# Fagear/SDVPCMdecoder

Measured on AMD Instinct MI355X. Metric: decoded video frames/sec (720x486 STC-007), binarize+bit-extract+CRC, bit-exact vs CPU, higher is better.
Workload: dtype u8; 1 GPU; configs[1]: 10000-frame synthetic STC-007 NTSC 720x486 batch per GPU resident in HBM, Binarizer mode 2, noise sigma 4.0, binarize+bit-extract+CRC only; decoded_words_match_generator=True

## Files before the change

### sdvpcmdecoder_amd/csrc/stc007_device.h

```cpp
#ifndef SDV_STC007_DEVICE_H
#define SDV_STC007_DEVICE_H

#include "../../include/sdvpcm.h"

#ifndef SDV_EMU
#include <hip/hip_runtime.h>
#endif

#define SDV_MAX_WIDTH 1536
#ifndef SDV_BATCH_LINES
#define SDV_BATCH_LINES 2
#endif
#ifndef SDV_NT_RECORDS
#define SDV_NT_RECORDS 1
#endif
#ifndef SDV_CAPTURE_D
#define SDV_CAPTURE_D 4
#endif
#ifndef SDV_RB_GENERAL
#define SDV_RB_GENERAL 1
#endif
#ifndef SDV_PREFETCH_ITERS
#define SDV_PREFETCH_ITERS 1
#endif
// ... 2015 lines not shown
    const int lane = lane_id();
    uint16_t w[9];
    bits_to_words(fb.s_lo, fb.s_hi, w);
    w[8] = fb.calc_crc;

    K1_T(t_bk0);
    const bool even_line = (line_num % 2) == 0;
    const bool doubled = a.doubled != 0;
    bool forced_bad = false;
    if (v.field_state == FIELD_NEW) v.field_state = FIELD_UNSAFE;
    v.good_coords_in_field++;
    v.q_line_length = (uint16_t)a.width;
    if (a.check_line_copy) {
        if (v.field_state == FIELD_UNSAFE) {
            b.in_coord.doubled = doubled;
            if (kMeasure) bin_set_bw_levels(b, ps, black, white);
            if (ps.en_first_line_dup) forced_bad = true;
        } else {
            uint8_t diff = words_diff_bit_count(w, v.last_words);
            Line t; t.m2 = a.m2_format != 0; for (int i = 0; i < 6; i++) t.words[i] = w[i];
            if (!stc_is_almost_silent(t) && diff <= (BITS_DATA / BIT_DIFF_THRES_DIV)) { forced_bad = true; if (!even_line) v.q_dup_odd++; else v.q_dup_even++; }
        }
    }
    K1_T(t_bk1);
    {
        uint32_t key = coords_key(b.in_coord.start, b.in_coord.stop);
        SDV_WAVE_SYNC();
        if (lane == 0) {
            if (v.n_last == COORD_HISTORY_DEPTH) for (int i = 0; i < COORD_HISTORY_DEPTH - 1; i++) lds.lv_keys[i] = lds.lv_keys[i + 1];
            lds.lv_keys[v.n_last == COORD_HISTORY_DEPTH ? COORD_HISTORY_DEPTH - 1 : v.n_last] = key;
        }
        if (v.n_last < COORD_HISTORY_DEPTH) v.n_last++;
        SDV_WAVE_SYNC();
        fv_keys[v.nfv++] = key;
        K1_T(t_bk2);
        K1_ADD(16, t_bk0, t_bk1); K1_ADD(17, t_bk1, t_bk2);
        if (a.coordinate_damper && (v.n_last > (COORD_HISTORY_DEPTH / 2))) {
            Coords target; coords_clear(target);
            uint32_t k;
            if (median_keys(lds.lv_keys, v.n_last, &k)) target = key_to_coords(k, false);
            if (!coords_valid(target)) target = v.frame_avg;
            if (coords_valid(target)) {
                int16_t ds = (int16_t)(b.in_coord.start - target.start), de = (int16_t)(b.in_coord.stop - target.stop);
                uint8_t in_delta = (uint8_t)(((uint8_t)(g.psm / 128u)) * 3);
                if (((int)ds <= -(int)in_delta) || ((int)ds >= (int)in_delta) || ((int)de <= -(int)in_delta) || ((int)de >= (int)in_delta)) forced_bad = true;
            }
        }
        K1_T(t_bk2b);
        K1_ADD(18, t_bk2, t_bk2b);
    }
    K1_T(t_bk3);
    if (!forced_bad) { b.in_coord.doubled = doubled; if (kMeasure) bin_set_bw_levels(b, ps, black, white); }
    else { if (!even_line) v.q_bad_odd++; else v.q_bad_even++; }
    v.field_state = FIELD_INIT;
    if (!even_line) { v.q_odd++; v.q_pcm_odd++; } else { v.q_even++; v.q_pcm_even++; }
    v.pcm_lines_in_field++;
    for (int i = 0; i < 8; i++) v.last_words[i] = w[i];
    v.line_in_field_cnt++;
    b.line_length = (uint16_t)a.width;

    if (lane == 0) {
        sdv_line_rec r;
        r.frame_number = frame_no; r.line_number = line_num;
        for (int i = 0; i < 9; i++) r.words[i] = w[i];
        r.calc_crc = fb.calc_crc;
        r.data_start = b.in_coord.start; r.data_stop = b.in_coord.stop;
        r.marker_start_bg_coord = 0; r.marker_start_ed_coord = 0; r.marker_stop_ed_coord = found_sp_ed;
        r.black_level = black; r.white_level = white; r.ref_low = fb.ref_low; r.ref_level = b.in_ref; r.ref_high = fb.ref_high;
        r.hysteresis_depth = fb.h; r.shift_stage = fb.s; r.service_type = SDV_SRV_NO;
        r.mark_st_stage = MARK_ST_START; r.mark_ed_stage = found_mark_ed;
        r.flags = (uint8_t)(SDV_LF_BY_EXT_TUNE | SDV_LF_BW_SET | (forced_bad ? SDV_LF_FORCED_BAD : SDV_LF_CRC_VALID) | (doubled ? SDV_LF_FROM_DOUBLED : 0));
        r.word_state = forced_bad ? 0 : (uint8_t)(SDV_WS_WORD_CRC | SDV_WS_WORD_VALID);
        *rec = r;
    }
    K1_T(t_bk4);
    K1_ADD(19, t_bk3, t_bk4);
    return true;
}

struct BatchLaneOut { uint64_t s_lo, s_hi; uint16_t crc; };
#ifdef SDV_EMU
__device__ __forceinline__ uint32_t write_lane(uint32_t old, uint32_t val, int lane) { return lane_id() == lane ? val : old; }
__device__ __forceinline__ uint8_t stream_load_u8(const uint8_t *p) { return *p; }
#define SDV_ISSUE_AFTER8(oa, ob, m0, m1, m2, m3, m4, m5, m6, m7) ((void)0)
#else
__device__ __forceinline__ uint8_t stream_load_u8(const uint8_t *p) { return __builtin_nontemporal_load(p); }
#define SDV_ISSUE_AFTER8(oa, ob, m0, m1, m2, m3, m4, m5, m6, m7) \
    asm volatile("" : "+s"(oa), "+s"(ob) : "s"(m0), "s"(m1), "s"(m2), "s"(m3), "s"(m4), "s"(m5), "s"(m6), "s"(m7))
extern "C" __device__ uint32_t sdv_llvm_writelane(uint32_t val, uint32_t lane, uint32_t old) __asm("llvm.amdgcn.writelane.i32");
__device__ __forceinline__ uint32_t write_lane(uint32_t old, uint32_t val, int lane) { return sdv_llvm_writelane(val, (uint32_t)lane, old); }
#endif
struct CaptureRaw { uint32_t a0, a1, a2, a3, b0, b1, b2, b3; };
__device__ __forceinline__ void capture_park(CaptureRaw &r, uint64_t a_lo, uint64_t a_hi, uint64_t b_lo, uint64_t b_hi, int j)
{
    r.a0 = write_lane(r.a0, (uint32_t)a_lo, j); r.a1 = write_lane(r.a1, (uint32_t)(a_lo >> 32), j);
    r.a2 = write_lane(r.a2, (uint32_t)a_hi, j); r.a3 = write_lane(r.a3, (uint32_t)(a_hi >> 32), j);
    r.b0 = write_lane(r.b0, (uint32_t)b_lo, j); r.b1 = write_lane(r.b1, (uint32_t)(b_lo >> 32), j);
    r.b2 = write_lane(r.b2, (uint32_t)b_hi, j); r.b3 = write_lane(r.b3, (uint32_t)(b_hi >> 32), j);
}
template <bool kAnyPattern = false>
__device__ inline bool capture_solve(const CaptureRaw &r, BatchLaneOut &o)
{
    const uint64_t a_lo = (uint64_t)r.a0 | ((uint64_t)r.a1 << 32), a_hi = (uint64_t)r.a2 | ((uint64_t)r.a3 << 32);
    const uint64_t b_lo = (uint64_t)r.b0 | ((uint64_t)r.b1 << 32), b_hi = (uint64_t)r.b2 | ((uint64_t)r.b3 << 32);
    const uint64_t e_lo = ~(a_lo ^ b_lo), e_hi = ~(a_hi ^ b_hi), t_lo = a_lo & ~b_lo, t_hi = a_hi & ~b_hi;
    const uint64_t pt_lo = prefix_xor64(t_lo), pt_hi = prefix_xor64(t_hi) ^ ((__popcll(t_lo) & 1) ? ~0ull : 0ull);
    const uint64_t u_lo = ((a_lo & b_lo) ^ pt_lo) & e_lo, u_hi = ((a_hi & b_hi) ^ pt_hi) & e_hi;
    const uint64_t x_lo = u_lo | ~e_lo, x_hi = u_hi | ~e_hi;
    const uint64_t y_lo = x_lo + u_lo, y_hi = x_hi + u_hi + ((y_lo < x_lo) ? 1ull : 0ull);
    const uint64_t s_lo = ((((y_lo ^ x_lo) & ~e_lo) | u_lo) ^ pt_lo), s_hi = ((((y_hi ^ x_hi) & ~e_hi) | u_hi) ^ pt_hi);
    uint32_t crc = 0;
#pragma unroll
    for (int j = 0; j < 16; j++) crc |= (uint32_t)((__popcll(s_lo & c_crc.klo[j]) + __popcll(s_hi & c_crc.khi[j])) & 1) << j;
    crc ^= c_crc.init;
    o.s_lo = s_lo; o.s_hi = s_hi; o.crc = (uint16_t)crc;
    return (uint16_t)crc == rev16((uint32_t)((s_hi >> 48) & 0xFFFF)) && (kAnyPattern || !ctrl_block_maybe(s_lo));
}

struct SolveOut { uint32_t d0, d1, d2, d3, crc_reads; };
#ifndef SDV_EMU
__device__ __attribute__((noinline)) SolveOut capture_solve_call(uint32_t a0, uint32_t a1, uint32_t a2, uint32_t a3, uint32_t b0, uint32_t b1, uint32_t b2, uint32_t b3)
#else
__device__ inline SolveOut capture_solve_call(uint32_t a0, uint32_t a1, uint32_t a2, uint32_t a3, uint32_t b0, uint32_t b1, uint32_t b2, uint32_t b3)
#endif
{
    CaptureRaw c; c.a0 = a0; c.a1 = a1; c.a2 = a2; c.a3 = a3; c.b0 = b0; c.b1 = b1; c.b2 = b2; c.b3 = b3;
    BatchLaneOut o;
    const bool reads = capture_solve<true>(c, o);
    SolveOut r; r.d0 = (uint32_t)o.s_lo; r.d1 = (uint32_t)(o.s_lo >> 32); r.d2 = (uint32_t)o.s_hi; r.d3 = (uint32_t)(o.s_hi >> 32);
    r.crc_reads = (uint32_t)o.crc | (reads ? 0x10000u : 0u);
    return r;
}

struct BatchLane { uint32_t d0, d1, d2, d3, meta; };

__device__ inline bool batch_eligible(const FrameArgs &a, const WaveLds &lds, const V2D &v, const Geo &g)
{
    if (!fast_eligible(a, v.bin)) return false;
    if (v.n_last != COORD_HISTORY_DEPTH) return false;
    uint32_t key = coords_key(v.bin.in_coord.start, v.bin.in_coord.stop);
    bool differs = (lane_id() < COORD_HISTORY_DEPTH) && (lds.lv_keys[lane_id() < COORD_HISTORY_DEPTH ? lane_id() : 0] != key);
    if (__ballot(differs) != 0ull) return false;
    if (a.coordinate_damper) {
        uint32_t psm = (uint32_t)((int)v.bin.in_coord.stop - (int)v.bin.in_coord.start);
        psm = (psm * 128u + BITS_BETWEEN / 2) / BITS_BETWEEN;
        if ((uint8_t)(((uint8_t)(psm / 128u)) * 3) == 0) return false;
    }
    return true;
}

enum { REC_STAGE_OFS = 5120, REC_STAGE_BYTES = 1024 };
static_assert(REC_STAGE_OFS >= ((SDV_MAX_HEIGHT / 2 + 63) / 64) * 4 * 64 * sizeof(uint32_t), "the parked lines of a field of SDV_MAX_HEIGHT / 2 lines end in front of the record stage");
static_assert(REC_STAGE_OFS >= SDV_PX_BYTES && REC_STAGE_OFS + REC_STAGE_BYTES <= offsetof(WaveLds, crc_stats), "the record stage lies behind the staged scanlines and in front of the histories");
#ifndef SDV_COALESCED_RECORDS
#define SDV_COALESCED_RECORDS 1
#endif

__device__ inline void batch_finish(const FrameArgs &a, WaveLds &lds, V2D &v, const BatchLane &bl, int n, uint32_t frame_no, uint16_t first_line_num,
                                    uint32_t *fv_keys, sdv_line_rec *rec, bool write_keys = true, uint4 *direct_dst = nullptr, int *n_forced = nullptr)
{
    const sdv_bin_preset &ps = a.preset;
    Bin &b = v.bin;
    const int lane = lane_id();
    const bool active = lane < n;
    const bool doubled = a.doubled != 0;
    const bool even_line = (first_line_num % 2) == 0;
    uint64_t s_lo = (uint64_t)bl.d0 | ((uint64_t)bl.d1 << 32), s_hi = (uint64_t)bl.d2 | ((uint64_t)bl.d3 << 32);
    uint16_t w[8];
    bits_to_words(s_lo, s_hi, w);
// ... 170 lines not shown
            v2d_give_up(a, lds, f);
            return;
        } else {
            uint16_t ln = 0;
            if (f == a.new_file_frame) { v2d_service_line(v, a, lds, wl, frame_no, 0, SDV_SRV_NEW_FILE); emit_record(wl, rec++); }
            for (int field = 0; field < 2; field++) {
                const int nl = field == 0 ? (a.height + 1) / 2 : a.height / 2;
                for (int i = 0; i < nl; i++) {
                    ln = (uint16_t)(field + 1 + 2 * i);
                    SDV_SLOW_CTX(c);
                    SDV_WAVE_SYNC();
                    if (!sc_args_set) { c.a = a; sc_args_set = true; }
                    c.v = v;
                    SDV_WAVE_SYNC();
                    empty_line(&c, &lds, frame_no, ln, fv_keys, fi_keys, rec++);
                    SDV_WAVE_SYNC();
                    v = c.v;
                    v2d_make_uniform(v);
                }
                ln = (uint16_t)(ln + 2);
                v2d_service_line(v, a, lds, wl, frame_no, ln, SDV_SRV_END_FIELD);
                emit_record(wl, rec++);
            }
            ln = (uint16_t)(ln + 2);
            v2d_service_line(v, a, lds, wl, frame_no, ln, SDV_SRV_END_FRAME);
            v2d_end_frame(v, a, lds, frame_no, fv_keys, fi_keys, &a.stats[f]);
            emit_record(wl, rec++);
            v2d_store_state(v, lds, &a.states_out[f], a);
            return;
        }
    }
    if (f == a.end_file_frame) {
        uint16_t ln = 0;
        for (int field = 0; field < 2; field++) {
            const int nl = field == 0 ? (a.height + 1) / 2 : a.height / 2;
            for (int i = 0; i < nl; i++) {
                ln = (uint16_t)(field + 1 + 2 * i);
                v2d_service_line(v, a, lds, wl, frame_no, ln, SDV_SRV_FILLER);
                emit_record(wl, rec++);
            }
            ln = (uint16_t)(ln + 2);
            v2d_service_line(v, a, lds, wl, frame_no, ln, SDV_SRV_END_FIELD);
            emit_record(wl, rec++);
        }
        ln = (uint16_t)(ln + 2);
        v2d_service_line(v, a, lds, wl, frame_no, ln, SDV_SRV_END_FILE);
        emit_record(wl, rec++);
        ln = (uint16_t)(ln + 2);
        v2d_service_line(v, a, lds, wl, frame_no, ln, SDV_SRV_END_FRAME);
        v2d_end_frame(v, a, lds, frame_no, fv_keys, fi_keys, &a.stats[f]);
        emit_record(wl, rec++);
        v2d_store_state(v, lds, &a.states_out[f], a);
        return;
    }
    if (f == a.new_file_frame) { v2d_service_line(v, a, lds, wl, frame_no, 0, SDV_SRV_NEW_FILE); emit_record(wl, rec++); }
    if (kFat && a.tc_hdr && lane == 0) a.tc_hdr[2 * f] = 0;
    if (!kLean && kMeet && a.tc_hdr) {
        tc_on = true;
        tc_prev = uniu(a.tc_hdr[2 * f]); tc_prev_n = uniu(a.tc_hdr[2 * f + 1]);
        if (tc_prev > 2u || tc_prev_n > (uint32_t)TC_FINAL) tc_prev = 0;
        tc_wbuf = tc_prev == 1u ? 1 : 0;
        tc_wr = a.tc_snaps + ((size_t)f * 2u + (size_t)tc_wbuf) * TC_ENTRIES;
        if (tc_prev) {
            tc_rd = a.tc_snaps + ((size_t)f * 2u + (size_t)(tc_prev - 1u)) * TC_ENTRIES;
            tc_my_pos = lane < (int)tc_prev_n ? (tc_rd[lane].d[18] & 0xFFFFu) : (uint32_t)TC_POS_NONE;
            tc_rd_keys = (tc_prev == 2u ? a.tc_keys : a.scratch) + (size_t)f * 2u * (size_t)a.height;
        }
        if (tc_wbuf) { fv_keys = a.tc_keys + (size_t)f * 2u * (size_t)a.height; fi_keys = fv_keys + a.height; }
        SDV_WAVE_SYNC();
        if (lane == 0) a.tc_hdr[2 * f] = 0;
    }
    const int n_field[2] = { (a.height + 1) / 2, a.height / 2 };
    RowPrefetch pf;
    pf.v0 = uint4{0, 0, 0, 0}; pf.v1 = uint4{0, 0, 0, 0};
    for (int u = 0; u < SDV_ROWQ; u++) { pf.vq[u] = uint4{0, 0, 0, 0}; pf.rowq[u] = frame; }
    pf.nq = 0;
    pf.vec = ((((uintptr_t)frame) | (uintptr_t)a.row_stride) & 15) == 0 && a.width >= 16;
    { int nvec = a.width >> 4; pf.i0 = lane < nvec ? lane : (nvec > 0 ? nvec - 1 : 0); }
    row_prefetch(pf, frame, a.width);
    const size_t row_step = 2 * a.row_stride;
    uint16_t line_num = 0;
    int start_field = 0, start_idx = 0;
    bool all_captured = false; uint32_t captured_key = 0;
    bool frame_direct = false;
    bool sweep_pending = false;
    bool used_general = false;
#ifdef SDV_K1_STAMPS
    int n_slow_lines = 0;
#endif
    if (kLean && pf.vec && a.width <= 1024 && (a.width & 15) == 0 && n_field[1] > 0 && (uint64_t)a.row_stride * (uint64_t)a.height < (1ull << 31) &&
        batch_eligible(a, lds, v, geo)) {
        const FastPre pre = fast_pre(a, v.bin, geo);
        if (pre.ok) {
            K1_T(t_cap);
            const int n0 = n_field[0], n1 = n_field[1];
            const int n_chunks = (n0 + 63) / 64;
            uint32_t *park = (uint32_t *)lds.px;
            uint64_t ok0_packed = 0, ok1_packed = 0;
            enum { HOLD_CHUNKS = (SDV_MAX_HEIGHT / 2 + 63) / 64 };
            uint32_t hold[HOLD_CHUNKS][4];
#pragma unroll
            for (int u = 0; u < HOLD_CHUNKS; u++) hold[u][0] = hold[u][1] = hold[u][2] = hold[u][3] = 0;
            int n_done = 0;
            const uint32_t rs = (uint32_t)a.row_stride;
            const uint32_t lo = pre.ref_low, hi = pre.ref_high;
            const uint32_t x0 = (uint32_t)pre.x0, x1 = (uint32_t)pre.x1;
            constexpr int D = SDV_CAPTURE_D;
            static_assert(64 % D == 0, "the prefetch queue must stay aligned with the 64-line chunks");
            auto pair_offsets = [&](int kn, uint32_t &oa, uint32_t &ob) {
                const uint32_t k = (uint32_t)(kn < n0 ? kn : n0 - 1);
                oa = 2u * k * rs; ob = (int)k < n1 ? oa + rs : oa; };
            uint8_t q[D][4];
#pragma unroll
            for (int d = 0; d < D; d++) {
                uint32_t oa, ob; pair_offsets(d, oa, ob);
                q[d][0] = stream_load_u8(frame + (oa + x0)); q[d][1] = stream_load_u8(frame + (oa + x1));
                q[d][2] = stream_load_u8(frame + (ob + x0)); q[d][3] = stream_load_u8(frame + (ob + x1));
            }
            bool whole = true;
            for (int c = 0; c < n_chunks && whole; c++) {
                const int cn0 = n0 - 64 * c < 64 ? n0 - 64 * c : 64, cn1 = n1 - 64 * c < 64 ? (n1 - 64 * c > 0 ? n1 - 64 * c : 0) : 64;
                CaptureRaw r0, r1;
                r0.a0 = r0.a1 = r0.a2 = r0.a3 = r0.b0 = r0.b1 = r0.b2 = r0.b3 = 0;
                r1 = r0;
                for (int j0 = 0; j0 < cn0; j0 += D) {
#pragma unroll
                    for (int d = 0; d < D; d++) {
                        const int j = j0 + d;
                        const uint8_t p0 = q[d][0], p1 = q[d][1], p2 = q[d][2], p3 = q[d][3];
                        const uint64_t aA_lo = __ballot(p0 > lo), bA_lo = __ballot(p0 >= hi), aA_hi = __ballot(p1 > lo), bA_hi = __ballot(p1 >= hi);
                        const uint64_t aB_lo = __ballot(p2 > lo), bB_lo = __ballot(p2 >= hi), aB_hi = __ballot(p3 > lo), bB_hi = __ballot(p3 >= hi);
                        {
                            uint32_t oa, ob; pair_offsets(64 * c + j + D, oa, ob);
                            SDV_ISSUE_AFTER8(oa, ob, aA_lo, bA_lo, aA_hi, bA_hi, aB_lo, bB_lo, aB_hi, bB_hi);
                            q[d][0] = stream_load_u8(frame + (oa + x0)); q[d][1] = stream_load_u8(frame + (oa + x1));
                            q[d][2] = stream_load_u8(frame + (ob + x0)); q[d][3] = stream_load_u8(frame + (ob + x1));
                        }
                        capture_park(r0, aA_lo, aA_hi, bA_lo, bA_hi, j);
                        capture_park(r1, aB_lo, aB_hi, bB_lo, bB_hi, j);
                    }
                }
                K1_T(t_s0);
                BatchLaneOut o0, o1;
                const bool ok0 = capture_solve(r0, o0), ok1 = capture_solve(r1, o1);
                const uint64_t okm0 = __ballot(ok0 || lane >= cn0), okm1 = __ballot(ok1 || lane >= cn1);
                const int n_ok0 = okm0 == ~0ull ? cn0 : (__ffsll((unsigned long long)~okm0) - 1);
                const int n_ok1 = okm1 == ~0ull ? cn1 : (__ffsll((unsigned long long)~okm1) - 1);
                ok0_packed |= (uint64_t)n_ok0 << (7 * c); ok1_packed |= (uint64_t)n_ok1 << (7 * c);
                K1_T(t_s1);
                K1_ADD(5, t_s0, t_s1);
                park[(c * 4 + 0) * 64 + lane] = (uint32_t)o1.s_lo; park[(c * 4 + 1) * 64 + lane] = (uint32_t)(o1.s_lo >> 32);
                park[(c * 4 + 2) * 64 + lane] = (uint32_t)o1.s_hi; park[(c * 4 + 3) * 64 + lane] = (uint32_t)(o1.s_hi >> 32);
#pragma unroll
                for (int u = 0; u < HOLD_CHUNKS; u++)
                    if (c == u) { hold[u][0] = (uint32_t)o0.s_lo; hold[u][1] = (uint32_t)(o0.s_lo >> 32); hold[u][2] = (uint32_t)o0.s_hi; hold[u][3] = (uint32_t)(o0.s_hi >> 32); }
                n_done = c + 1;
                if (n_ok0 < cn0) { whole = false; start_field = 0; start_idx = 64 * c + n_ok0; }
            }
            bool direct = false;
            if (a.direct_fields && whole && f + 1 < a.n_total && f != a.new_file_frame && n0 <= a.direct_lines && n1 <= a.direct_lines) {
                direct = true;
                for (int c = 0; c < n_chunks; c++) {
                    const int cn1 = n1 - 64 * c < 64 ? (n1 - 64 * c > 0 ? n1 - 64 * c : 0) : 64;
                    if ((int)((ok1_packed >> (7 * c)) & 0x7F) != cn1) direct = false;
                }
            }
            uint4 *const dfield0 = direct ? (uint4 *)a.direct_fields + ((size_t)(f + a.direct_seg_ofs) * 2u) * (size_t)a.direct_pitch * 2u : nullptr;
            uint4 *const dfield1 = direct ? dfield0 + (size_t)a.direct_pitch * 2u : nullptr;
            int forced0 = 0, forced1 = 0;
            K1_T(t_s1b);
            for (int c = 0; c < n_done; c++) {
                const int n_ok0 = (int)((ok0_packed >> (7 * c)) & 0x7F);
                BatchLane bl; bl.d0 = bl.d1 = bl.d2 = bl.d3 = 0;
#pragma unroll
                for (int u = 0; u < HOLD_CHUNKS; u++)
                    if (c == u) { bl.d0 = hold[u][0]; bl.d1 = hold[u][1]; bl.d2 = hold[u][2]; bl.d3 = hold[u][3]; }
                bl.meta = (uint32_t)rev16(bl.d3 >> 16);
                int nf = 0;
                if (n_ok0 > 0) { batch_finish(a, lds, v, bl, n_ok0, frame_no, (uint16_t)(1 + 2 * (64 * c)), fv_keys, rec, false, direct ? dfield0 + 128 * c : nullptr, &nf); rec += n_ok0; }
                forced0 += nf;
            }
            K1_T(t_s2);
            K1_ADD(6, t_s1b, t_s2);
            if (whole) {
                line_num = (uint16_t)(1 + 2 * n0);
                v2d_service_line(v, a, lds, wl, frame_no, line_num, SDV_SRV_END_FIELD);
                if (!direct) emit_record(wl, rec);
                rec++;
                start_field = 1; start_idx = 0;
                SDV_WAVE_SYNC();
                for (int c = 0; c < n_chunks && whole; c++) {
                    const int cn1 = n1 - 64 * c < 64 ? (n1 - 64 * c > 0 ? n1 - 64 * c : 0) : 64;
                    if (cn1 <= 0) break;
                    const int n_ok1 = (int)((ok1_packed >> (7 * c)) & 0x7F);
                    BatchLane bl;
                    bl.d0 = park[(c * 4 + 0) * 64 + lane]; bl.d1 = park[(c * 4 + 1) * 64 + lane]; bl.d2 = park[(c * 4 + 2) * 64 + lane];
                    bl.d3 = park[(c * 4 + 3) * 64 + lane]; bl.meta = (uint32_t)rev16(bl.d3 >> 16);
                    int nf = 0;
                    if (n_ok1 > 0) { batch_finish(a, lds, v, bl, n_ok1, frame_no, (uint16_t)(2 + 2 * (64 * c)), fv_keys, rec, false, direct ? dfield1 + 128 * c : nullptr, &nf); rec += n_ok1; }
                    forced1 += nf;
                    if (n_ok1 < cn1) { whole = false; start_idx = 64 * c + n_ok1; }
                }
                SDV_WAVE_SYNC();
                if (whole) {
                    line_num = (uint16_t)(2 + 2 * n1);
                    v2d_service_line(v, a, lds, wl, frame_no, line_num, SDV_SRV_END_FIELD);
                    if (!direct) emit_record(wl, rec);
                    rec++;
                    start_field = 2;
                    all_captured = true; captured_key = coords_key(v.bin.in_coord.start, v.bin.in_coord.stop);
                    frame_direct = direct;
                    if (direct) {
                        dsum.frame_number = frame_no; dsum.n[0] = (uint16_t)n0; dsum.n[1] = (uint16_t)n1; dsum.bad[0] = (uint16_t)forced0; dsum.bad[1] = (uint16_t)forced1;
                        dsum.ref = v.bin.in_ref; dsum.flag = 1;
                    }
                }
            }
            if (start_field < 2) {
                const uint32_t key = coords_key(v.bin.in_coord.start, v.bin.in_coord.stop);
#pragma unroll 1
                for (int i = lane; i < v.nfv; i += 64) fv_keys[i] = key;
                pf.nq = 0;
                row_prefetch(pf, frame + (size_t)(2 * start_idx + start_field) * a.row_stride, a.width);
            }
            K1_T(t_cap1);
            K1_ADD(4, t_cap, t_cap1);
        }
    }
    bool stop_frame = false;
    int last_miss_field = -1, last_miss_idx = 0;
    bool sticky_rung = false; int first_rung_run = 0;
    int calm_lines = 0;
    int rb_lines = 16;
    int rung_hint = 0;
    auto tc_point = [&](uint32_t pos) -> bool {
        if (!tc_on) return false;
        if (tc_w < TC_FINAL) { tc_write(tc_wr + tc_w, v, lds, pos, used_general); tc_w++; }
        if (!tc_prev) return false;
        const uint64_t at_m = __ballot(tc_my_pos == pos);
        if (at_m == 0ull) return false;
        const int r = __ffsll((unsigned long long)at_m) - 1;
        const uint32_t theirs = lane < TC_SNAP_DWORDS ? tc_rd[r].d[lane < TC_SNAP_DWORDS ? lane : 0] : 0u;
        const uint32_t mine = tc_dword(v, lds, lane < TC_USED_DWORDS ? lane : 0, pos, used_general);
#if defined(SDV_EMU) && defined(SDV_DEV_AIDS)
        if (getenv("SDV_TC_DEBUG")) {
            const uint64_t dm = __ballot(lane < TC_CMP_DWORDS && mine != theirs);
            if (lane == 0) fprintf(stderr, "[tc] frame %d pos %u: differing dwords %05llx%s\n", f, pos, (unsigned long long)dm, dm ? "" : "  -> met");
            if (dm && ((dm >> lane) & 1)) fprintf(stderr, "[tc]    dword %d: now %08x, last pass %08x\n", lane, mine, theirs);
        }
#endif
        if (__ballot(lane < TC_CMP_DWORDS && mine != theirs) != 0ull) return false;
        uint32_t *const stg = lds.hist;
        SDV_WAVE_SYNC();
        if (lane < TC_SNAP_DWORDS) { stg[lane] = theirs; stg[TC_SNAP_DWORDS + lane] = tc_rd[TC_FINAL].d[lane]; }
        SDV_WAVE_SYNC();
        const TcCounts was = tc_counts(stg), fin = tc_counts(stg + TC_SNAP_DWORDS);
#pragma unroll 1
        for (int i = was.nfv + lane; i < fin.nfv; i += 64) fv_keys[v.nfv + (i - was.nfv)] = tc_rd_keys[i];
#pragma unroll 1
        for (int i = was.nfi + lane; i < fin.nfi; i += 64) fi_keys[v.nfi + (i - was.nfi)] = tc_rd_keys[a.height + i];
        {
            const uint32_t d_lo = (mine & 0xFFFFu) - (theirs & 0xFFFFu), d_hi = (mine >> 16) - (theirs >> 16);
            const bool counted = lane >= 19 && lane < TC_USED_DWORDS;
#pragma unroll 1
            for (int e = r + 1; e < (int)tc_prev_n && tc_w < TC_FINAL; e++) {
                uint32_t x = lane < TC_SNAP_DWORDS ? tc_rd[e].d[lane < TC_SNAP_DWORDS ? lane : 0] : 0u;
                if (counted) x = (((x & 0xFFFFu) + d_lo) & 0xFFFFu) | ((((x >> 16) + d_hi) & 0xFFFFu) << 16);
                if (lane == 18 && used_general) x |= 0x10000u;
                if (lane < TC_USED_DWORDS) tc_wr[tc_w].d[lane] = x;
                tc_w++;
            }
        }
        v.nfv += fin.nfv - was.nfv; v.nfi += fin.nfi - was.nfi;
        if (fin.q[0] > v.q_line_length) v.q_line_length = fin.q[0];
        v.q_odd = (uint16_t)(v.q_odd + fin.q[1] - was.q[1]); v.q_even = (uint16_t)(v.q_even + fin.q[2] - was.q[2]);
        v.q_pcm_odd = (uint16_t)(v.q_pcm_odd + fin.q[3] - was.q[3]); v.q_pcm_even = (uint16_t)(v.q_pcm_even + fin.q[4] - was.q[4]);
        v.q_bad_odd = (uint16_t)(v.q_bad_odd + fin.q[5] - was.q[5]); v.q_bad_even = (uint16_t)(v.q_bad_even + fin.q[6] - was.q[6]);
        v.q_dup_odd = (uint16_t)(v.q_dup_odd + fin.q[7] - was.q[7]); v.q_dup_even = (uint16_t)(v.q_dup_even + fin.q[8] - was.q[8]);
        used_general = used_general || fin.used_general;
        const uint32_t *const fs = stg + TC_SNAP_DWORDS;
        v.n_last = (int)((fs[16] >> 8) & 0xFFu); v.field_state = (uint8_t)(fs[16] & 0xFFu);
        SDV_WAVE_SYNC();
        if (lane < COORD_HISTORY_DEPTH) lds.lv_keys[lane] = fs[lane];
        SDV_WAVE_SYNC();
        for (int i = 0; i < 4; i++) { v.last_words[2 * i] = (uint16_t)fs[9 + i]; v.last_words[2 * i + 1] = (uint16_t)(fs[9 + i] >> 16); }
        v.bin.in_coord.start = (int16_t)(uint16_t)fs[13]; v.bin.in_coord.stop = (int16_t)(uint16_t)(fs[13] >> 16);
        v.bin.in_black = (uint8_t)fs[15]; v.bin.in_white = (uint8_t)(fs[15] >> 8); v.bin.in_ref = (uint8_t)(fs[15] >> 16);
        v.bin.in_coord.doubled = ((fs[15] >> 24) & 1u) != 0; v.bin.do_ref_lvl_sweep = ((fs[15] >> 24) & 2u) != 0;
        v2d_make_uniform(v);
        if (lane == 0 && a.memo_count) atomicAdd(a.memo_count + 1, 1);
        return true;
    };
    bool tc_due = !kLean && kMeet && tc_on;
    for (int field = start_field; field < 2 && !stop_frame && !tc_met; field++) {
        const int nl = n_field[field];
        int idx = field == start_field ? start_idx : 0;
        while (idx < nl && !stop_frame && !tc_met) {
            if (!kLean && kMeet && tc_due) { tc_due = false; if (tc_point((uint32_t)(field * 1024 + idx))) { tc_met = true; break; } }
            bool staged = false, batch_gave_way = false;
            FastPre pre; pre.ok = false;
            if (pf.vec && a.width <= 1024 && (a.width & 15) == 0 && batch_eligible(a, lds, v, geo)) pre = fast_pre(a, v.bin, geo);
            if (pre.ok) {
                K1_T(t_batch);
                int nb = nl - idx; if (nb > 64) nb = 64;
                BatchLane bl; bl.d0 = bl.d1 = bl.d2 = bl.d3 = bl.meta = 0;
                int j = 0;
                bool redo = false;
                auto row_in_order = [&](int k) -> const uint8_t * {
                    if (k < nl) return frame + (size_t)(2 * k + field) * a.row_stride;
                    if (field == 0 && (k - nl) < n_field[1]) return frame + (size_t)(2 * (k - nl) + 1) * a.row_stride;
                    return frame;
                };
                if ((kLean || (kMeet && SDV_RB_GENERAL && calm_lines >= 48)) && sticky_rung && rung_hint >= 1 && rung_hint <= SHIFT_STAGES_MAX && rung_hint <= (int)v.bin.in_max_shift) {
                    const int n_rungs = rung_hint + 1;
                    enum { RB_OFS = 1024, RB_SLOTS = (REC_STAGE_OFS + REC_STAGE_BYTES - RB_OFS) / 32 };
                    static_assert(RB_OFS + RB_SLOTS * 32 <= offsetof(WaveLds, crc_stats), "the parked masks end in front of the histories");
                    uint4 *const rb = (uint4 *)((uint8_t *)&lds + RB_OFS);
// ... 380 lines not shown
```

Before: 14.96 million frames/s.

## Add shift-rung batch capture path to keep lines on fast path after capture failures

When the fast batched capture fails on a chunk, the kernel now probes whether a shifted sampling position (shift stages 1-2) would decode the failing line. If so, it re-runs capture from that chunk with 32-bit unaligned loads covering neighboring pixels, solving all shift stages per line and recording the chosen stage per chunk in the metadata passed to batch_finish. It also seeds the later slow per-line path with a sticky rung hint. The aim is to avoid falling back to the slow general per-line path on shifted/noisy frames, at the cost of extra ballots, registers and more solve work per line.

```diff
diff --git a/sdvpcmdecoder_amd/csrc/stc007_device.h b/sdvpcmdecoder_amd/csrc/stc007_device.h
--- a/sdvpcmdecoder_amd/csrc/stc007_device.h
+++ b/sdvpcmdecoder_amd/csrc/stc007_device.h
@@ -2121,9 +2121,12 @@
 #ifdef SDV_EMU
 __device__ __forceinline__ uint32_t write_lane(uint32_t old, uint32_t val, int lane) { return lane_id() == lane ? val : old; }
 __device__ __forceinline__ uint8_t stream_load_u8(const uint8_t *p) { return *p; }
+__device__ __forceinline__ uint32_t stream_load_u32(const uint8_t *p) { uint32_t w; __builtin_memcpy(&w, p, 4); return w; }
 #define SDV_ISSUE_AFTER8(oa, ob, m0, m1, m2, m3, m4, m5, m6, m7) ((void)0)
 #else
 __device__ __forceinline__ uint8_t stream_load_u8(const uint8_t *p) { return __builtin_nontemporal_load(p); }
+typedef uint32_t sdv_u32_any_align __attribute__((aligned(1)));
+__device__ __forceinline__ uint32_t stream_load_u32(const uint8_t *p) { return __builtin_nontemporal_load((const sdv_u32_any_align *)p); }
 #define SDV_ISSUE_AFTER8(oa, ob, m0, m1, m2, m3, m4, m5, m6, m7) \
     asm volatile("" : "+s"(oa), "+s"(ob) : "s"(m0), "s"(m1), "s"(m2), "s"(m3), "s"(m4), "s"(m5), "s"(m6), "s"(m7))
 extern "C" __device__ uint32_t sdv_llvm_writelane(uint32_t val, uint32_t lane, uint32_t old) __asm("llvm.amdgcn.writelane.i32");
@@ -2460,6 +2463,7 @@
     uint16_t line_num = 0;
     int start_field = 0, start_idx = 0;
     bool all_captured = false; uint32_t captured_key = 0;
+    int rung_seed = 0;
     bool frame_direct = false;
     bool sweep_pending = false;
     bool used_general = false;
@@ -2496,6 +2500,10 @@
                 q[d][2] = stream_load_u8(frame + (ob + x0)); q[d][3] = stream_load_u8(frame + (ob + x1));
             }
             bool whole = true;
+            const bool rung_ok = v.bin.in_max_shift >= 1 &&
+                                 __ballot(geo.vp0 < 1 || geo.vp1 < 1 || geo.vp0 + 2 > a.width - 2 || geo.vp1 + 2 > a.width - 2) == 0ull;
+            int rung_from = -1;
+            uint32_t hold_stage = 0, park_stage = 0;
             for (int c = 0; c < n_chunks && whole; c++) {
                 const int cn0 = n0 - 64 * c < 64 ? n0 - 64 * c : 64, cn1 = n1 - 64 * c < 64 ? (n1 - 64 * c > 0 ? n1 - 64 * c : 0) : 64;
                 CaptureRaw r0, r1;
@@ -2524,6 +2532,25 @@
                 const uint64_t okm0 = __ballot(ok0 || lane >= cn0), okm1 = __ballot(ok1 || lane >= cn1);
                 const int n_ok0 = okm0 == ~0ull ? cn0 : (__ffsll((unsigned long long)~okm0) - 1);
                 const int n_ok1 = okm1 == ~0ull ? cn1 : (__ffsll((unsigned long long)~okm1) - 1);
+                if (rung_ok && (n_ok0 < cn0 || n_ok1 < cn1)) {
+                    const bool in_f0 = n_ok0 < cn0;
+                    const uint32_t o = (2u * (uint32_t)(64 * c + (in_f0 ? n_ok0 : n_ok1)) + (in_f0 ? 0u : 1u)) * rs;
+                    const uint32_t w0 = stream_load_u32(frame + (o + x0 - 1u)), w1 = stream_load_u32(frame + (o + x1 - 1u));
+                    const int s_end = v.bin.in_max_shift >= 2 ? 3 : 2;
+                    bool later = false;
+#pragma unroll 1
+                    for (int s = 1; s < s_end && !later; s++) {
+                        const int sh = s == 1 ? 16 : 0;
+                        const uint32_t p0 = (w0 >> sh) & 0xFFu, p1 = (w1 >> sh) & 0xFFu;
+                        const uint64_t a_lo = __ballot(p0 > lo), a_hi = __ballot(p1 > lo), b_lo = __ballot(p0 >= hi), b_hi = __ballot(p1 >= hi);
+                        CaptureRaw m;
+                        m.a0 = (uint32_t)a_lo; m.a1 = (uint32_t)(a_lo >> 32); m.a2 = (uint32_t)a_hi; m.a3 = (uint32_t)(a_hi >> 32);
+                        m.b0 = (uint32_t)b_lo; m.b1 = (uint32_t)(b_lo >> 32); m.b2 = (uint32_t)b_hi; m.b3 = (uint32_t)(b_hi >> 32);
+                        BatchLaneOut bo;
+                        later = capture_solve(m, bo);
+                    }
+                    if (later) { rung_from = c; break; }
+                }
                 ok0_packed |= (uint64_t)n_ok0 << (7 * c); ok1_packed |= (uint64_t)n_ok1 << (7 * c);
                 K1_T(t_s1);
                 K1_ADD(5, t_s0, t_s1);
@@ -2534,6 +2561,100 @@
                     if (c == u) { hold[u][0] = (uint32_t)o0.s_lo; hold[u][1] = (uint32_t)(o0.s_lo >> 32); hold[u][2] = (uint32_t)o0.s_hi; hold[u][3] = (uint32_t)(o0.s_hi >> 32); }
                 n_done = c + 1;
                 if (n_ok0 < cn0) { whole = false; start_field = 0; start_idx = 64 * c + n_ok0; }
+            }
+            if (rung_from >= 0) {
+                int S = (int)v.bin.in_max_shift + 1; if (S > 3) S = 3;
+                const uint32_t xm0 = x0 - 1u, xm1 = x1 - 1u;
+                uint32_t w[D][4];
+#pragma unroll
+                for (int d = 0; d < D; d++) {
+                    uint32_t oa, ob; pair_offsets(64 * rung_from + d, oa, ob);
+                    w[d][0] = stream_load_u32(frame + (oa + xm0)); w[d][1] = stream_load_u32(frame + (oa + xm1));
+                    w[d][2] = stream_load_u32(frame + (ob + xm0)); w[d][3] = stream_load_u32(frame + (ob + xm1));
+                }
+                static_assert(32 % D == 0, "the prefetch queue must stay aligned with the 32-pair chunks");
+                for (int c = rung_from; c < n_chunks && whole; c++) {
+                    int nk0 = 0, nk1 = 0;
+                    for (int h = 0; h < 2 && whole; h++) {
+                        const int base = 64 * c + 32 * h;
+                        const int cn0 = n0 - base < 32 ? n0 - base : 32, cn1 = n1 - base < 32 ? (n1 - base > 0 ? n1 - base : 0) : 32;
+                        if (cn0 <= 0) break;
+                        const int l0 = 32 * h, l1 = 32 - l0;
+                        CaptureRaw R[3];
+#pragma unroll
+                        for (int s = 0; s < 3; s++) R[s].a0 = R[s].a1 = R[s].a2 = R[s].a3 = R[s].b0 = R[s].b1 = R[s].b2 = R[s].b3 = 0;
+                        for (int j0 = 0; j0 < cn0; j0 += D) {
+#pragma unroll
+                            for (int d = 0; d < D; d++) {
+                                const int j = j0 + d;
+                                const uint32_t wa0 = w[d][0], wa1 = w[d][1], wb0 = w[d][2], wb1 = w[d][3];
+#pragma unroll
+                                for (int s = 2; s >= 1; s--)
+                                    if (s < S) {
+                                        const int sh = s == 1 ? 16 : 0;
+                                        const uint32_t p0 = (wa0 >> sh) & 0xFFu, p1 = (wa1 >> sh) & 0xFFu, p2 = (wb0 >> sh) & 0xFFu, p3 = (wb1 >> sh) & 0xFFu;
+                                        capture_park(R[s], __ballot(p0 > lo), __ballot(p1 > lo), __ballot(p0 >= hi), __ballot(p1 >= hi), l0 + j);
+                                        capture_park(R[s], __ballot(p2 > lo), __ballot(p3 > lo), __ballot(p2 >= hi), __ballot(p3 >= hi), l1 + j);
+                                    }
+                                const uint32_t p0 = (wa0 >> 8) & 0xFFu, p1 = (wa1 >> 8) & 0xFFu, p2 = (wb0 >> 8) & 0xFFu, p3 = (wb1 >> 8) & 0xFFu;
+                                const uint64_t aA_lo = __ballot(p0 > lo), bA_lo = __ballot(p0 >= hi), aA_hi = __ballot(p1 > lo), bA_hi = __ballot(p1 >= hi);
+                                const uint64_t aB_lo = __ballot(p2 > lo), bB_lo = __ballot(p2 >= hi), aB_hi = __ballot(p3 > lo), bB_hi = __ballot(p3 >= hi);
+                                {
+                                    uint32_t oa, ob; pair_offsets(base + j + D, oa, ob);
+                                    SDV_ISSUE_AFTER8(oa, ob, aA_lo, bA_lo, aA_hi, bA_hi, aB_lo, bB_lo, aB_hi, bB_hi);
+                                    w[d][0] = stream_load_u32(frame + (oa + xm0)); w[d][1] = stream_load_u32(frame + (oa + xm1));
+                                    w[d][2] = stream_load_u32(frame + (ob + xm0)); w[d][3] = stream_load_u32(frame + (ob + xm1));
+                                }
+                                capture_park(R[0], aA_lo, aA_hi, bA_lo, bA_hi, l0 + j);
+                                capture_park(R[0], aB_lo, aB_hi, bB_lo, bB_hi, l1 + j);
+                            }
+                        }
+                        int my_rung = -1; BatchLaneOut mine; mine.s_lo = mine.s_hi = 0; mine.crc = 0;
+#pragma unroll 1
+                        for (int s = 0; s < S; s++) {
+                            CaptureRaw m = R[0];
+                            if (s == 1) m = R[1];
+                            if (s == 2) m = R[2];
+                            BatchLaneOut o;
+                            const bool reads = capture_solve<true>(m, o);
+                            if (my_rung < 0 && reads) { my_rung = s; mine = o; }
+                        }
+                        const bool f0_lane = (lane >> 5) == h;
+                        const int jl = lane & 31;
+                        const bool taken = my_rung >= 0 && !ctrl_block_maybe(mine.s_lo);
+                        const uint64_t taken_m = __ballot(taken || jl >= (f0_lane ? cn0 : cn1));
+                        const uint32_t tm0 = (uint32_t)(taken_m >> l0), tm1 = (uint32_t)(taken_m >> l1);
+                        const int k0 = tm0 == ~0u ? cn0 : (__ffsll((unsigned long long)(uint32_t)~tm0) - 1);
+                        const int k1 = tm1 == ~0u ? cn1 : (__ffsll((unsigned long long)(uint32_t)~tm1) - 1);
+#if defined(SDV_EMU) && defined(SDV_DEV_AIDS)
+                        if (lane == 0 && getenv("SDV_RB_DEBUG")) fprintf(stderr, "[rc] frame %d pairs %d ..: %d of %d + %d of %d lines taken on %d stages\n", f, base, k0, cn0, k1, cn1, S);
+#endif
+                        const uint32_t stage = my_rung > 0 ? (uint32_t)my_rung : 0u;
+                        const uint32_t stage_f1 = (uint32_t)__shfl((int)stage, lane ^ 32);
+                        if (f0_lane) {
+                            hold_stage = (hold_stage & ~(3u << (2 * c))) | (stage << (2 * c));
+                            park_stage = (park_stage & ~(3u << (2 * c))) | (stage_f1 << (2 * c));
+#pragma unroll
+                            for (int u = 0; u < HOLD_CHUNKS; u++)
+                                if (c == u) { hold[u][0] = (uint32_t)mine.s_lo; hold[u][1] = (uint32_t)(mine.s_lo >> 32); hold[u][2] = (uint32_t)mine.s_hi; hold[u][3] = (uint32_t)(mine.s_hi >> 32); }
+                        } else {
+                            park[(c * 4 + 0) * 64 + l0 + jl] = (uint32_t)mine.s_lo; park[(c * 4 + 1) * 64 + l0 + jl] = (uint32_t)(mine.s_lo >> 32);
+                            park[(c * 4 + 2) * 64 + l0 + jl] = (uint32_t)mine.s_hi; park[(c * 4 + 3) * 64 + l0 + jl] = (uint32_t)(mine.s_hi >> 32);
+                        }
+                        if (h == 0) { nk0 = k0; nk1 = k1; } else { nk0 += k0; if (nk1 == 32) nk1 += k1; }
+                        {
+                            const bool counted = taken && jl < (f0_lane ? k0 : k1);
+                            const int n_taken = __popcll(__ballot(counted));
+                            const int top = __ballot(counted && my_rung == 2) != 0ull ? 2 : (__ballot(counted && my_rung == 1) != 0ull ? 1 : 0);
+                            if (n_taken >= 8 && top < S - 1) S = top + 1;
+                        }
+                        if (k0 < cn0) whole = false;
+                    }
+                    ok0_packed |= (uint64_t)nk0 << (7 * c); ok1_packed |= (uint64_t)nk1 << (7 * c);
+                    n_done = c + 1;
+                    if (!whole) { start_field = 0; start_idx = 64 * c + nk0; }
+                }
+                rung_seed = S - 1;
             }
             bool direct = false;
             if (a.direct_fields && whole && f + 1 < a.n_total && f != a.new_file_frame && n0 <= a.direct_lines && n1 <= a.direct_lines) {
@@ -2553,7 +2674,7 @@
 #pragma unroll
                 for (int u = 0; u < HOLD_CHUNKS; u++)
                     if (c == u) { bl.d0 = hold[u][0]; bl.d1 = hold[u][1]; bl.d2 = hold[u][2]; bl.d3 = hold[u][3]; }
-                bl.meta = (uint32_t)rev16(bl.d3 >> 16);
+                bl.meta = (uint32_t)rev16(bl.d3 >> 16) | (((hold_stage >> (2 * c)) & 3u) << 20);
                 int nf = 0;
                 if (n_ok0 > 0) { batch_finish(a, lds, v, bl, n_ok0, frame_no, (uint16_t)(1 + 2 * (64 * c)), fv_keys, rec, false, direct ? dfield0 + 128 * c : nullptr, &nf); rec += n_ok0; }
                 forced0 += nf;
@@ -2573,7 +2694,7 @@
                     const int n_ok1 = (int)((ok1_packed >> (7 * c)) & 0x7F);
                     BatchLane bl;
                     bl.d0 = park[(c * 4 + 0) * 64 + lane]; bl.d1 = park[(c * 4 + 1) * 64 + lane]; bl.d2 = park[(c * 4 + 2) * 64 + lane];
-                    bl.d3 = park[(c * 4 + 3) * 64 + lane]; bl.meta = (uint32_t)rev16(bl.d3 >> 16);
+                    bl.d3 = park[(c * 4 + 3) * 64 + lane]; bl.meta = (uint32_t)rev16(bl.d3 >> 16) | (((park_stage >> (2 * c)) & 3u) << 20);
                     int nf = 0;
                     if (n_ok1 > 0) { batch_finish(a, lds, v, bl, n_ok1, frame_no, (uint16_t)(2 + 2 * (64 * c)), fv_keys, rec, false, direct ? dfield1 + 128 * c : nullptr, &nf); rec += n_ok1; }
                     forced1 += nf;
@@ -2611,6 +2732,7 @@
     int calm_lines = 0;
     int rb_lines = 16;
     int rung_hint = 0;
+    if (kLean && rung_seed > 0 && start_field < 2) { sticky_rung = true; rung_hint = rung_seed; rb_lines = 64; }
     auto tc_point = [&](uint32_t pos) -> bool {
         if (!tc_on) return false;
         if (tc_w < TC_FINAL) { tc_write(tc_wr + tc_w, v, lds, pos, used_general); tc_w++; }
```

Result: slower. 14.14 million frames/s (-5.5%).
